# thoglu/jammy_flows

Measured on AMD Instinct MI355X. Metric: log-prob evals/sec (batch 2^20), e4+s2+e4 / gggg+f+gggg, higher is better.
Workload: dtype f32; 1 GPU; pdf("e4+s2+e4","gggg+f+gggg") log-prob, unconditional pdf with autoregressive conditioning, 1048576 rows in total, row-sharded; batch_per_gpu=1048576, total_rows=1048576, parallelism=rows sharded over 1 GPU(s)

## Files before the change

jammy_flows_amd/csrc/jf_cond_regs.h:

```cpp
#pragma once
#include <type_traits>
#include "jf_gf.h"

namespace jf {

using bf16x8 = __attribute__((ext_vector_type(8))) __bf16;
typedef __attribute__((address_space(3))) void* cs_lptr;
typedef const __attribute__((address_space(1))) void* cs_gptr;

constexpr int CS_K = 10;
constexpr int CS_HH = 4;
constexpr int CS_SLOTS = 36;
constexpr int CS_SLOT_MEAN = 0, CS_SLOT_LW = CS_K, CS_SLOT_LN = 2 * CS_K, CS_SLOT_ROT = 3 * CS_K, CS_SLOT_OFF = 3 * CS_K + CS_HH;
struct CsLayer { int hh, model_offset, inv_type; float wmin, inv_wmax, nmin, nmax; };

struct CsPackLayer { int col0, off_rot, off_mean, off_lw, off_ln, hh, model_offset; };
__device__ __forceinline__ int cs_slot_column(const CsPackLayer& o, int D, int slot, int d) {
    if (d >= D) return -1;
    if (slot < CS_SLOT_LW) return o.off_mean + slot * D + d;
    if (slot < CS_SLOT_LN) return o.off_lw + (slot - CS_SLOT_LW) * D + d;
    if (slot < CS_SLOT_ROT) return o.off_ln + (slot - CS_SLOT_LN) * D + d;
    if (slot < CS_SLOT_OFF) return (slot - CS_SLOT_ROT) < o.hh ? o.off_rot + (slot - CS_SLOT_ROT) * D + d : -1;
    if (slot == CS_SLOT_OFF) return o.model_offset ? d : -1;
    return -1;
}

__device__ __forceinline__ void cs_split(float v, __bf16& hi, __bf16& mid, __bf16& lo) {
    hi = (__bf16)v;
    const float r1 = v - (float)hi;
    mid = (__bf16)r1;
    lo = (__bf16)(r1 - (float)mid);
}

constexpr float CS_M_SCALED = 60.0f;

struct CsSums { float C, S, P, invN; };
__device__ __forceinline__ MixQ<float> cs_mixture(const float (&P)[CS_SLOTS], const CsLayer& o, float x, bool live, CsSums* sums = nullptr) {
    using Mf = M<float>;
    float iw[CS_K], wk[CS_K], u[CS_K];
    float m = INFINITY, Nn = 0.f;
#pragma unroll
    for (int k = 0; k < CS_K; ++k) {
        const float ae = o.inv_wmax + Mf::exp_fast(-P[CS_SLOT_LW + k]);
        iw[k] = ae * Mf::rcp(o.wmin * ae + 1.0f);
        wk[k] = o.nmin + o.nmax * Mf::rcp(1.0f + Mf::exp_fast(-P[CS_SLOT_LN + k]));
        u[k] = (x - P[CS_SLOT_MEAN + k]) * iw[k];
        m = fminf(m, fabsf(u[k]));
        Nn += wk[k];
    }
    const float inv = Mf::rcp(Nn);
    MixQ<float> q;
    {
        float C = 0.f, S = 0.f, Pd = 0.f;
#pragma unroll
        for (int k = 0; k < CS_K; ++k) {
            const float t = Mf::exp_fast(fminf(-u[k], 87.0f));
            const float s = Mf::rcp(1.0f + t);
            const float ts = t * s;
            C += wk[k] * s;
            S += wk[k] * ts;
            Pd += wk[k] * s * ts * iw[k];
        }
        C *= inv; S *= inv; Pd *= inv;
        q.lc = Mf::log_fast(C); q.ls = Mf::log_fast(S); q.lp = Mf::log_fast(Pd);
        q.cdf = C; q.sf = S;
        if (sums) *sums = CsSums{C, S, Pd, inv};
    }
    const bool far = m > CS_M_SCALED;
    if (!__any(live && far)) return q;
    const float em = Mf::exp_fast(-m);
    float Cu = 0.f, Cs = 0.f, Su = 0.f, Ss = 0.f, Ps = 0.f;
#pragma unroll
    for (int k = 0; k < CS_K; ++k) {
        const float t = Mf::exp_fast(m - fabsf(u[k]));
        const float hi = Mf::rcp(1.0f + t * em);
        const float c1 = wk[k] * hi, c2 = c1 * t;
        if (u[k] >= 0.f) { Cu += c1; Ss += c2; }
        else { Su += c1; Cs += c2; }
        Ps += c2 * hi * iw[k];
    }
    Cu *= inv; Cs *= inv; Su *= inv; Ss *= inv; Ps *= inv;
    if (far) {
        q.cdf = Cu + em * Cs;
        q.sf = Su + em * Ss;
        q.lc = Cu > 0.f ? Mf::log_fast(q.cdf) : Mf::log_fast(Cs) - m;
        q.ls = Su > 0.f ? Mf::log_fast(q.sf) : Mf::log_fast(Ss) - m;
        q.lp = Mf::log_fast(Ps) - m;
        if (sums) *sums = CsSums{q.cdf, q.sf, Ps * em, inv};
    }
    return q;
}

__device__ __forceinline__ void cs_derive(float (&P)[CS_SLOTS], const CsLayer& o) {
    using Mf = M<float>;
    float Nn = 0.f;
#pragma unroll
    for (int k = 0; k < CS_K; ++k) {
        const float ae = o.inv_wmax + Mf::exp_fast(-P[CS_SLOT_LW + k]);
        P[CS_SLOT_LW + k] = ae * Mf::rcp(o.wmin * ae + 1.0f);
        const float w = o.nmin + o.nmax * Mf::rcp(1.0f + Mf::exp_fast(-P[CS_SLOT_LN + k]));
        P[CS_SLOT_LN + k] = w;
        Nn += w;
    }
    const float inv = Mf::rcp(Nn);
#pragma unroll
    for (int k = 0; k < CS_K; ++k) P[CS_SLOT_LN + k] *= inv;
}

template <typename T> __device__ __forceinline__ MixQ<T> cs_mixture_derived(const T (&P)[CS_SLOTS], T x) {
    using Mf = M<T>;
    T C = T(0), S = T(0), Pd = T(0);
#pragma unroll
    for (int k = 0; k < CS_K; ++k) {
        const T iw = P[CS_SLOT_LW + k], wk = P[CS_SLOT_LN + k];
        const T u = (x - P[CS_SLOT_MEAN + k]) * iw;
        if constexpr (sizeof(T) == 4) {
            const T t = Mf::exp_fast(Mf::min(-u, T(87)));
            const T s = Mf::rcp(T(1) + t);
            const T ts = t * s;
            C += wk * s;
            S += wk * ts;
            Pd += wk * s * ts * iw;
        } else {
            const T t = Mf::exp_fast(-Mf::abs(u));
            const T hi = Mf::rcp(T(1) + t);
            const T lo = t * hi;
            const bool pos = u >= T(0);
            C += wk * (pos ? hi : lo);
            S += wk * (pos ? lo : hi);
            Pd += wk * hi * lo * iw;
        }
    }
    MixQ<T> q;
    q.lc = Mf::log_fast(C); q.ls = Mf::log_fast(S); q.lp = Mf::log_fast(Pd);
    q.cdf = C; q.sf = S;
    const bool under = !(C > Mf::TINY && S > Mf::TINY && Pd > Mf::TINY);
    if (__any(under)) {
        T m = T(INFINITY);
#pragma unroll
        for (int k = 0; k < CS_K; ++k) m = Mf::min(m, Mf::abs((x - P[CS_SLOT_MEAN + k]) * P[CS_SLOT_LW + k]));
        const T em = Mf::exp_fast(-m);
        T Cu = T(0), Cs = T(0), Su = T(0), Ss = T(0), Ps = T(0);
#pragma unroll
        for (int k = 0; k < CS_K; ++k) {
            const T iw = P[CS_SLOT_LW + k], wk = P[CS_SLOT_LN + k];
            const T u = (x - P[CS_SLOT_MEAN + k]) * iw;
            const T t = Mf::exp_fast(m - Mf::abs(u));
            const T hi = Mf::rcp(T(1) + t * em);
            const T c1 = wk * hi, c2 = c1 * t;
            if (u >= T(0)) { Cu += c1; Ss += c2; }
            else { Su += c1; Cs += c2; }
            Ps += c2 * hi * iw;
        }
        if (under) {
            q.cdf = Cu + em * Cs;
            q.sf = Su + em * Ss;
            q.lc = Cu > T(0) ? Mf::log_fast(q.cdf) : Mf::log_fast(Cs) - m;
            q.ls = Su > T(0) ? Mf::log_fast(q.sf) : Mf::log_fast(Ss) - m;
            q.lp = Mf::log_fast(Ps) - m;
        }
    }
    return q;
}

struct CsSolveInfo { int steps; bool nonconv, nonfinite; };
template <typename T, typename RSUM, typename RMAX>
__device__ __forceinline__ T cs_solve(const T (&P)[CS_SLOTS], int inv_type, bool live, T z, bool row_valid, bool leader, int32_t* status,
                                      RSUM rsum, RMAX rmax, CsSolveInfo* info = nullptr, T* logd_out = nullptr, bool have_start = false, T start = T(0)) {
    using Mf = M<T>;
    using F = typename std::conditional<sizeof(T) == 8, float, T>::type;
    T x = have_start ? start : T(0);
    if (__any(live && !have_start)) {
        F PF[CS_SLOTS];
#pragma unroll
        for (int k = 0; k < CS_SLOTS; ++k) PF[k] = k < 3 * CS_K ? (F)P[k] : F(0);
        F xf = F(0), wbar = F(0), m2 = F(0);
#pragma unroll
        for (int k = 0; k < CS_K; ++k) {
            const F pm = PF[CS_SLOT_LN + k] * PF[CS_SLOT_MEAN + k];
            xf += pm;
            m2 += pm * PF[CS_SLOT_MEAN + k];
            wbar += PF[CS_SLOT_LN + k] * M<F>::rcp(PF[CS_SLOT_LW + k]);
        }
        {
            const F zc = M<F>::min(M<F>::max((F)z, F(-8)), F(8));
            const F var_b = M<F>::max(m2 - xf * xf, F(0));
            const F sc = inv_type != JF_GF_ISIGMOID ? M<F>::sqrt(F(2.896804) * wbar * wbar + var_b) : M<F>::sqrt(wbar * wbar + F(0.30396355) * var_b);
            xf += sc * zc;
        }
#ifdef JF_PROBE_COUNT_APPROACH
        int n_ev = 0;
        xf = gf_approach<F>([&](F xx) { return cs_mixture_derived<F>(PF, xx); }, inv_type != JF_GF_ISIGMOID, (F)z, xf, live && !have_start, &n_ev);
        if (info == nullptr) { for (int i = 0; i < n_ev; ++i) status_add(status, JF_STATUS_NEWTON_STEPS, row_valid && leader); }
#else
        xf = gf_approach<F>([&](F xx) { return cs_mixture_derived<F>(PF, xx); }, inv_type != JF_GF_ISIGMOID, (F)z, xf, live && !have_start);
#endif
        if (!have_start) x = (T)xf;
    }
    bool active = row_valid;
    T ferr = T(0), prev = T(INFINITY);
    bool nonfinite = false;
    int n_steps = 0;
    T last_logd = T(0);
    bool coarse_end = false;
    for (int it = 0; it < 20 && __any(active); ++it) {
        const IcdfOut<T> s = gf_icdf<T>(inv_type, cs_mixture_derived<T>(P, x));
        const T f = s.y - z;
        T upd;
        if constexpr (sizeof(T) == 4) upd = f * Mf::exp_fast(-s.logd);
        else upd = f / Mf::exp(s.logd);
        const T usum = rsum(live ? Mf::abs(upd) : T(0));
        if (info == nullptr) status_add(status, JF_STATUS_NEWTON_STEPS, active && leader);
        n_steps += active ? 1 : 0;
        if (active) {
            const T nx = x - upd;
            if (Mf::finite(nx)) x = nx; else nonfinite = nonfinite || live;
            ferr = Mf::abs(f);
            last_logd = s.logd;
            active = usum >= newton_tol<T>();
        }
        if (sizeof(T) == 4 && !newton_reference_rule()) {
            const T xs = rsum(live ? Mf::max(Mf::abs(x), T(1)) : T(0));
            const bool done = usum < T(2.5e-7) * xs || (usum < T(JF_F32_NEWTON_FLOOR) * xs && rmax(live ? Mf::abs(f) : T(0)) <= T(1e-4));
            if (active && usum >= T(0.5) * prev && usum < T(1e-4) * xs && !done) coarse_end = true;
            if (done || (usum >= T(0.5) * prev && usum < T(1e-4) * xs)) active = false;
            prev = usum;
        }
    }
    if (logd_out != nullptr) {
        const bool stale = row_valid && (active || n_steps == 0 || coarse_end);
        if (__any(stale)) *logd_out = gf_icdf<T>(inv_type, cs_mixture_derived<T>(P, x)).logd;
        else *logd_out = last_logd;
    }
    const T prec = sizeof(T) == 8 ? T(1e-7) : T(1e-4);
    const T ferr_row = rmax(live ? ferr : T(0));
    const T nf_row = rmax(nonfinite ? T(1) : T(0));
    if (info != nullptr) {
        info->steps = n_steps; info->nonconv = ferr_row > prec; info->nonfinite = nf_row > T(0);
        return x;
    }
    status_add(status, JF_STATUS_NONCONVERGED, row_valid && leader && (ferr_row > prec));
// ... 6 lines not shown
```

jammy_flows_amd/csrc/jf_cond_split.h:

```cpp
#pragma once
#include "jf_cond_in.h"
#include "jf_cond_regs.h"
#include "jf_mfma.h"

namespace jf {

constexpr int CS_TILES = 9;
static_assert(CS_SLOTS == 4 * CS_TILES, "one register per slot, four registers per tile");
constexpr int CS_CT = 3;
constexpr int CS_CPL = CS_TILES / CS_CT;
constexpr int CS_KSTEPS = 4;
constexpr int CS_NP = 3;
constexpr int CS_FRAG = 1024;
constexpr int CS_W_BYTES = CS_CT * CS_KSTEPS * CS_NP * CS_FRAG;
constexpr int CS_B_BYTES = CS_CT * 16 * 4;
constexpr int CS_CHUNK_BYTES = CS_W_BYTES + CS_B_BYTES;
constexpr int CS_NP16 = 2;
constexpr int CS_W16_BYTES = CS_CT * CS_KSTEPS * CS_NP16 * CS_FRAG;
constexpr int CS_B16_BYTES = CS_B_BYTES + 16;
constexpr int CS_CHUNK16_BYTES = CS_W16_BYTES + CS_B16_BYTES;
constexpr float CS_H_SCALE = 16384.0f;
using f16x8 = __attribute__((ext_vector_type(8))) _Float16;
using f16x2 = __attribute__((ext_vector_type(2))) _Float16;
using f32x2 = __attribute__((ext_vector_type(2))) float;
__device__ __forceinline__ int cs_w_exponent(float wmax) {
    if (!(wmax > 0.f && wmax < INFINITY)) return 0;
    const int e = 14 - ilogbf(wmax);
    return e < -60 ? -60 : (e > 60 ? 60 : e);
}
static __global__ void __launch_bounds__(1024) cs_absmax_kernel(const float* __restrict__ W, int64_t ws, int N, int H, float* __restrict__ out) {
    __shared__ float part[16];
    float m = 0.f;
    const int lane = threadIdx.x & 63, wave = threadIdx.x >> 6;
    if (H == 128 && ws % 4 == 0 && (reinterpret_cast<uintptr_t>(W) & 15u) == 0) {
        const int half = lane >> 5, l4 = (lane & 31) * 4;
        for (int n0 = 8 * wave; n0 < N; n0 += 128) {
            f32x4 v[4];
#pragma unroll
            for (int u = 0; u < 4; ++u) {
                const int n = n0 + 2 * u + half;
                v[u] = n < N ? *reinterpret_cast<const f32x4*>(W + (int64_t)n * ws + l4) : f32x4{0.f, 0.f, 0.f, 0.f};
            }
#pragma unroll
            for (int u = 0; u < 4; ++u) m = fmaxf(fmaxf(m, fmaxf(fabsf(v[u][0]), fabsf(v[u][1]))), fmaxf(fabsf(v[u][2]), fabsf(v[u][3])));
        }
    } else {
        for (int n0 = 4 * wave; n0 < N; n0 += 64) {
            for (int k = lane; k < H; k += 64) {
                float v[4];
#pragma unroll
                for (int u = 0; u < 4; ++u) v[u] = n0 + u < N ? W[(int64_t)(n0 + u) * ws + k] : 0.f;
#pragma unroll
                for (int u = 0; u < 4; ++u) m = fmaxf(m, fabsf(v[u]));
            }
        }
    }
#pragma unroll
    for (int o = 32; o > 0; o >>= 1) m = fmaxf(m, __shfl_xor(m, o));
    if ((threadIdx.x & 63) == 0) part[threadIdx.x >> 6] = m;
    __syncthreads();
    if (threadIdx.x < 4) {
        float t = 0.f;
        if (threadIdx.x == 0) {
#pragma unroll
            for (int w = 0; w < 16; ++w) t = fmaxf(t, part[w]);
        }
        out[threadIdx.x] = t;
    }
}
template <int NP> struct CsGeom;
template <> struct CsGeom<3> { static constexpr int W = CS_W_BYTES, B = CS_B_BYTES, CHUNK = CS_CHUNK_BYTES; };
template <> struct CsGeom<2> { static constexpr int W = CS_W16_BYTES, B = CS_B16_BYTES, CHUNK = CS_CHUNK16_BYTES; };
__device__ __forceinline__ void cs_split16(float v0, float v1, unsigned& hi, unsigned& lo) {
    const f16x2 h = __builtin_convertvector(f32x2{v0, v1}, f16x2);
    const f32x2 back = __builtin_convertvector(h, f32x2);
    const f16x2 l = __builtin_convertvector(f32x2{v0 - back[0], v1 - back[1]}, f16x2);
    hi = __builtin_bit_cast(unsigned, h);
    lo = __builtin_bit_cast(unsigned, l);
}
constexpr int CS_ROWS1 = 64;
constexpr int CS_HMAX = 128, CS_K1MAX = 28;

template <typename Op> __device__ __forceinline__ float cs_rreduce(float v, Op op) {
    float a = v, b = v;
    asm("s_nop 1\n\tv_permlane16_swap_b32 %0, %1" : "+v"(a), "+v"(b));
    float c = op(a, b), e = c;
    asm("s_nop 1\n\tv_permlane32_swap_b32 %0, %1" : "+v"(c), "+v"(e));
    return op(c, e);
}
__device__ __forceinline__ float cs_rsum(float v) { return cs_rreduce(v, [](float a, float b) { return a + b; }); }
__device__ __forceinline__ float cs_rmax(float v) { return cs_rreduce(v, [](float a, float b) { return fmaxf(a, b); }); }

static inline bool cs_layer_supported(const jf_gf_layer& h, int D) {
    return h.num_kde == CS_K && h.hh_iter >= 0 && h.hh_iter <= CS_HH && h.nonlinear_stretch_type == JF_GF_STRETCH_CLASSIC &&
           h.rotation_mode == JF_GF_ROT_HOUSEHOLDER && !h.center_mean && !h.add_skewness &&
           h.width_mode == JF_GF_WIDTH_SMOOTH_SATURATION && !h.clamp_widths && h.fit_normalization && h.regulate_normalization &&
           h.width_min > 0 && h.width_max > 0 && D >= 3 && D <= 4;
}

__device__ __forceinline__ void cs_dma_chunk(__amdgpu_buffer_rsrc_t rsrc, unsigned char* dst, int g, int lane_off, int wave, int lane, int w_bytes,
                                             int b_bytes) {
#pragma unroll
    for (int u = 0; u < CS_W_BYTES / 4096; ++u)
        if (u < w_bytes / 4096) __builtin_amdgcn_raw_ptr_buffer_load_lds(rsrc, (cs_lptr)(dst + (u * 4 + wave) * 1024), 16, lane_off, g + u * 4096, 0, 0);
    if (wave == 0 && lane < b_bytes / 16) __builtin_amdgcn_raw_ptr_buffer_load_lds(rsrc, (cs_lptr)(dst + w_bytes), 16, lane * 16, g + w_bytes, 0, 0);
}

template <int RG, bool STORE_H, int NP = CS_NP>
__device__ __forceinline__ void cs_hidden(const float* __restrict__ in, int64_t in_stride, const float* __restrict__ W1, int64_t w1s,
                                          const float* __restrict__ b1, int K1, int H, int64_t row0, int64_t last, float* Xs,
                                          bf16x8 (&hB)[RG][CS_KSTEPS][NP], float* __restrict__ h_out, int64_t hs, const CondIn* cin = nullptr) {
    using MF = Mfma16<float>;
    constexpr int CS_ROWS = CS_ROWS1 * RG;
    constexpr int MT = 16, KS = 4, NREG = 4, JH = CS_HMAX / MT;
    const int tid = threadIdx.x, lane = tid & 63, wave = tid >> 6;
    const int li = lane & 15, lq = lane >> 4;
    const int k1p = (K1 + KS - 1) / KS * KS, ldk = k1p + 1;
    float* W1s = Xs + CS_ROWS * ldk;
    float* b1s = W1s + CS_HMAX * ldk;
    {
        const int nx = CS_ROWS * k1p, nw = CS_HMAX * k1p;
        if (cin) {
            const bool any_embed = cond_in_any_embed(*cin);
            for (int base = 0; base < nx; base += 4 * 256) {
                CondLoc<float> loc[4]; float va[4], vb[4]; int o[4]; bool keep[4];
#pragma unroll
                for (int u = 0; u < 4; ++u) {
                    const int idx = base + u * 256 + tid;
                    const int r = idx / k1p, c = idx - r * k1p;
                    const int64_t gr = row0 + r;
                    loc[u] = cond_in_locate<float>(*cin, gr <= last ? gr : last, c < K1 ? c : 0);
                    keep[u] = c < K1;
                    o[u] = idx < nx ? r * ldk + c : -1;
                }
#pragma unroll
                for (int u = 0; u < 4; ++u) { va[u] = *loc[u].pa; vb[u] = *loc[u].pb; }
#pragma unroll
                for (int u = 0; u < 4; ++u) {
                    const float t = cond_in_finish<float, true>(loc[u], va[u], vb[u], any_embed);
                    if (o[u] >= 0) Xs[o[u]] = keep[u] ? t : 0.f;
                }
            }
        } else
        for (int base = 0; base < nx; base += 4 * 256) {
            float v[4]; int o[4];
#pragma unroll
            for (int u = 0; u < 4; ++u) {
                const int idx = base + u * 256 + tid;
                const int r = idx / k1p, c = idx - r * k1p;
                const int64_t gr = row0 + r;
                const float t = in[(gr <= last ? gr : last) * in_stride + (c < K1 ? c : 0)];
                v[u] = c < K1 ? t : 0.f;
                o[u] = idx < nx ? r * ldk + c : -1;
            }
#pragma unroll
            for (int u = 0; u < 4; ++u) if (o[u] >= 0) Xs[o[u]] = v[u];
        }
        for (int base = 0; base < nw; base += 4 * 256) {
            float v[4]; int o[4];
#pragma unroll
            for (int u = 0; u < 4; ++u) {
                const int idx = base + u * 256 + tid;
                const int r = idx / k1p, c = idx - r * k1p;
                const float t = W1[(int64_t)(r < H ? r : H - 1) * w1s + (c < K1 ? c : 0)];
                v[u] = (r < H && c < K1) ? t : 0.f;
                o[u] = idx < nw ? r * ldk + c : -1;
            }
#pragma unroll
            for (int u = 0; u < 4; ++u) if (o[u] >= 0) W1s[o[u]] = v[u];
        }
        if (tid < CS_HMAX) b1s[tid] = tid < H ? b1[tid < H ? tid : 0] : 0.f;
    }
    __syncthreads();
#pragma unroll
    for (int g = 0; g < RG; ++g) {
        typename MF::Acc acc[JH];
#pragma unroll
        for (int j = 0; j < JH; ++j)
#pragma unroll
            for (int r = 0; r < NREG; ++r) acc[j][r] = 0.f;
        for (int s = 0; s < k1p / KS; ++s) {
            const int kk = s * KS + lq;
            const float xb = Xs[((wave * RG + g) * MT + li) * ldk + kk];
#pragma unroll
            for (int j = 0; j < JH; ++j) acc[j] = MF::mma(W1s[(j * MT + li) * ldk + kk], xb, acc[j]);
        }
#pragma unroll
        for (int s = 0; s < CS_KSTEPS; ++s) {
            using u32x4 = __attribute__((ext_vector_type(4))) unsigned;
            u32x4 q0, q1, q2;
#pragma unroll
            for (int i = 0; i < 8; i += 2) {
                const int j = 2 * s + (i >> 2), r = i & 3;
                const float h0 = M<float>::tanh_fast(acc[j][r] + b1s[j * MT + 4 * lq + r]);
                const float h1 = M<float>::tanh_fast(acc[j][r + 1] + b1s[j * MT + 4 * lq + r + 1]);
                if constexpr (STORE_H) { acc[j][r] = h0; acc[j][r + 1] = h1; }
                if constexpr (NP == 2) {
                    unsigned ph, pl;
                    cs_split16(h0 * CS_H_SCALE, h1 * CS_H_SCALE, ph, pl);
                    q0[i >> 1] = ph; q1[i >> 1] = pl;
                    continue;
                }
                const unsigned a0 = __builtin_bit_cast(unsigned, h0), a1 = __builtin_bit_cast(unsigned, h1);
                const float r0 = h0 - __builtin_bit_cast(float, a0 & 0xffff0000u), r1 = h1 - __builtin_bit_cast(float, a1 & 0xffff0000u);
                const unsigned c0 = __builtin_bit_cast(unsigned, r0), c1 = __builtin_bit_cast(unsigned, r1);
                const float s0 = r0 - __builtin_bit_cast(float, c0 & 0xffff0000u), s1 = r1 - __builtin_bit_cast(float, c1 & 0xffff0000u);
                q0[i >> 1] = __builtin_amdgcn_perm(a1, a0, 0x07060302u);
                q1[i >> 1] = __builtin_amdgcn_perm(c1, c0, 0x07060302u);
                q2[i >> 1] = __builtin_amdgcn_perm(__builtin_bit_cast(unsigned, s1), __builtin_bit_cast(unsigned, s0), 0x07060302u);
            }
            hB[g][s][0] = __builtin_bit_cast(bf16x8, q0); hB[g][s][1] = __builtin_bit_cast(bf16x8, q1);
            if constexpr (NP == 3) hB[g][s][2] = __builtin_bit_cast(bf16x8, q2);
        }
        if constexpr (STORE_H) {
            const int64_t r = row0 + (wave * RG + g) * MT + li;
            if (r <= last) {
#pragma unroll
                for (int j = 0; j < JH; ++j) {
                    const int c = j * MT + 4 * lq;
                    if (c < H) *reinterpret_cast<f32x4*>(h_out + r * hs + c) = acc[j];
                }
            }
        }
    }
}

}
```

jammy_flows_amd/csrc/jf_cond_split_kernel.h:

```cpp
#pragma once
#include "jf_cond_split.h"

namespace jf {

constexpr int CS_MAX_PRE = 4;
struct CsArgs {
    const float* in; int64_t in_stride;
    const float* W1; int64_t w1s; const float* b1;
    const unsigned char* packed;
    int K1, H;
    const float* x; int64_t xs;
    const float* ld_in;
    int64_t B;
    int D, n_layers;
    CsLayer L[JF_MAX_CHAIN];
    float* x_out; int64_t xos;
    float* ld_out;
    const float* blp_in; float* blp_out;
    int32_t* status;
    float* aux;
    CondIn cin;
    const float* ld_pre[CS_MAX_PRE]; const float* blp_pre[CS_MAX_PRE];
    int n_ld_pre, n_blp_pre;
    float* total;
};

template <int RG, bool FWD, bool SAVE, int NP>
__device__ __forceinline__ void cond_gf_split_body(const CsArgs& a, const int block, unsigned char* smem_raw) {
    using G = CsGeom<NP>;
    constexpr int CS_ROWS = CS_ROWS1 * RG;
    constexpr int MT = 16;
    unsigned char* Ws0 = smem_raw;
    float* Xs = reinterpret_cast<float*>(smem_raw + G::CHUNK);
    const int tid = threadIdx.x, lane = tid & 63, wave = tid >> 6;
    const int li = lane & 15, lq = lane >> 4;
    const int64_t row0 = (int64_t)block * CS_ROWS;
    const int64_t last = a.B - 1;
    const int D = a.D;
    const __amdgpu_buffer_rsrc_t packed_rsrc =
        __builtin_amdgcn_make_buffer_rsrc(const_cast<unsigned char*>(a.packed), 0, a.n_layers * CS_CPL * G::CHUNK, 0x00027000);
    const int lane_off = wave * 1024 + lane * 16;
    auto dma = [&](int chunk) {
        const int img = FWD ? (a.n_layers - 1 - chunk / CS_CPL) * CS_CPL + chunk % CS_CPL : chunk;
        const int g = img * G::CHUNK;
        cs_dma_chunk(packed_rsrc, Ws0 + (chunk & 1) * G::CHUNK, g, lane_off, wave, lane, G::W, G::B);
    };
    dma(0);

    bf16x8 hB[RG][CS_KSTEPS][NP];
    cs_hidden<RG, false, NP>(a.in, a.in_stride, a.W1, a.w1s, a.b1, a.K1, a.H, row0, last, Xs, hB, nullptr, 0, a.cin.n ? &a.cin : nullptr);
    const bool live = lq < D, leader = lq == 0;
    int d = live ? lq : D - 1;
    int64_t row[RG]; bool row_valid[RG];
    float x[RG], ld[RG];
#pragma unroll
    for (int g = 0; g < RG; ++g) {
        row[g] = row0 + (wave * RG + g) * MT + li;
        row_valid[g] = row[g] <= last;
        const int64_t rrow = row_valid[g] ? row[g] : last;
        x[g] = a.x[rrow * a.xs + d];
        ld[g] = a.ld_in ? a.ld_in[rrow] : 0.f;
    }

    auto landed = [&]() { asm volatile("s_waitcnt vmcnt(0) lgkmcnt(0)\n\ts_barrier" ::: "memory"); };

    const int n_chunks = a.n_layers * CS_CPL;
    landed();
    int chunk = 0;
    for (int li = 0; li < a.n_layers; ++li) {
        const int l = FWD ? li : a.n_layers - 1 - li;
        float P[RG][CS_SLOTS];
#pragma unroll
        for (int c = 0; c < CS_CPL; ++c, ++chunk) {
            if (chunk + 1 < n_chunks) dma(chunk + 1);
            const unsigned char* Ws = Ws0 + (chunk & 1) * G::CHUNK;
            const float* Bs = reinterpret_cast<const float*>(Ws + G::W);
            f32x4 acc[RG][CS_CT];
#pragma unroll
            for (int t = 0; t < CS_CT; ++t) {
                const f32x4 bias = *reinterpret_cast<const f32x4*>(Bs + t * 16 + 4 * lq);
#pragma unroll
                for (int g = 0; g < RG; ++g) acc[g][t] = bias;
            }
            bf16x8 A[2][CS_CT][NP];
            auto load_a = [&](int s, int buf) {
#pragma unroll
                for (int t = 0; t < CS_CT; ++t)
#pragma unroll
                    for (int p = 0; p < NP; ++p)
                        A[buf][t][p] = *reinterpret_cast<const bf16x8*>(Ws + ((t * CS_KSTEPS + s) * NP + p) * CS_FRAG + lane * 16);
            };
            load_a(0, 0);
#pragma unroll
            for (int s = 0; s < CS_KSTEPS; ++s) {
                const int b = s & 1;
                if (s + 1 < CS_KSTEPS) load_a(s + 1, b ^ 1);
                if constexpr (NP == 3) {
                    constexpr int PA[6] = {2, 1, 0, 1, 0, 0}, PB[6] = {0, 1, 2, 0, 1, 0};
#pragma unroll
                    for (int i = 0; i < 6; ++i)
#pragma unroll
                        for (int t = 0; t < CS_CT; ++t)
#pragma unroll
                            for (int g = 0; g < RG; ++g)
                                acc[g][t] = __builtin_amdgcn_mfma_f32_16x16x32_bf16(A[b][t][PA[i]], hB[g][s][PB[i]], acc[g][t], 0, 0, 0);
                } else {
#pragma unroll
                    for (int i = 0; i < 3; ++i)
#pragma unroll
                        for (int t = 0; t < CS_CT; ++t)
#pragma unroll
                            for (int g = 0; g < RG; ++g) {
                                const f16x8 af = __builtin_bit_cast(f16x8, A[b][t][i == 0 ? 1 : 0]), bf = __builtin_bit_cast(f16x8, hB[g][s][i == 1 ? 1 : 0]);
                                acc[g][t] = __builtin_amdgcn_mfma_f32_16x16x32_f16(af, bf, acc[g][t], 0, 0, 0);
                            }
                }
            }
            if constexpr (NP == 3) {
#pragma unroll
                for (int g = 0; g < RG; ++g)
#pragma unroll
                    for (int t = 0; t < CS_CT; ++t)
#pragma unroll
                        for (int r = 0; r < 4; ++r) P[g][4 * (c * CS_CT + t) + r] = acc[g][t][r];
            } else {
                const float inv = Bs[CS_B_BYTES / 4];
#pragma unroll
                for (int g = 0; g < RG; ++g)
#pragma unroll
                    for (int t = 0; t < CS_CT; ++t)
#pragma unroll
                        for (int r = 0; r < 4; ++r) P[g][4 * (c * CS_CT + t) + r] = acc[g][t][r] * inv;
            }
            if (c + 1 < CS_CPL) landed();
        }
        const CsLayer o = a.L[l];
#pragma unroll
        for (int g = 0; g < RG; ++g) {
            if constexpr (!FWD) {
                float xg = x[g] - P[g][CS_SLOT_OFF];
#pragma unroll
                for (int i = 0; i < CS_HH; ++i) {
                    if (i < o.hh) {
                        const float v = live ? P[g][CS_SLOT_ROT + i] : 0.f;
                        const float n2 = cs_rsum(v * v), dot = cs_rsum(v * xg);
                        xg -= 2.0f * dot * M<float>::rcp(n2) * v;
                    }
                }
                CsSums sums;
                const MixQ<float> q = cs_mixture(P[g], o, xg, live, SAVE ? &sums : nullptr);
                if constexpr (SAVE) {
                    {
                        int t2 = tid;
                        asm volatile("" : "+v"(t2));
                        row[g] = row0 + ((t2 >> 6) * RG + g) * MT + (t2 & 15);
                        row_valid[g] = row[g] <= last;
                    }
                    if (row_valid[g]) {
                        const int64_t slot = ((int64_t)l * a.B + row[g]) * 4 + lq;
                        reinterpret_cast<f32x4*>(a.aux)[slot] = f32x4{sums.C, sums.S, sums.P, sums.invN};
                        a.aux[(int64_t)a.n_layers * a.B * 16 + slot] = x[g];
                    }
                }
                const IcdfOut<float> sy = gf_icdf<float>(o.inv_type, q);
                x[g] = sy.y;
                ld[g] += cs_rsum(live ? sy.logd : 0.f);
            } else {
                cs_derive(P[g], o);
                float slogd;
                float xs = cs_solve<float>(P[g], o.inv_type, live, x[g], row_valid[g], leader, a.status, [](float v) { return cs_rsum(v); },
                                    [](float v) { return cs_rmax(v); }, nullptr, &slogd);
                ld[g] -= cs_rsum(live ? slogd : 0.f);
#pragma unroll
                for (int i = CS_HH - 1; i >= 0; --i) {
                    if (i < o.hh) {
                        const float v = live ? P[g][CS_SLOT_ROT + i] : 0.f;
                        const float n2 = cs_rsum(v * v), dot = cs_rsum(v * xs);
                        xs -= 2.0f * dot * M<float>::rcp(n2) * v;
                    }
                }
                x[g] = xs + P[g][CS_SLOT_OFF];
            }
        }
        landed();
    }

    if constexpr (!FWD) {
        int t2 = tid;
        asm volatile("" : "+v"(t2));
        const int lane2 = t2 & 63, wave2 = t2 >> 6, li2 = lane2 & 15, lq2 = lane2 >> 4;
        d = lq2 < D ? lq2 : D - 1;
#pragma unroll
        for (int g = 0; g < RG; ++g) {
            row[g] = row0 + (wave2 * RG + g) * MT + li2;
            row_valid[g] = row[g] <= last;
        }
    }
#pragma unroll
    for (int g = 0; g < RG; ++g) {
        if (row_valid[g] && live) a.x_out[row[g] * a.xos + d] = x[g];
        if constexpr (FWD) {
            if (row_valid[g] && leader) a.ld_out[row[g]] = ld[g];
        } else {
            float sb = 0.f;
            if (a.blp_out) sb = cs_rsum(live ? -0.5f * x[g] * x[g] - M<float>::HALF_LN_2PI : 0.f);
            if (row_valid[g] && leader) {
                float ldv = ld[g], bv = sb + (a.blp_in ? a.blp_in[row[g]] : 0.f);
                if (a.n_ld_pre > 0) {
                    float t = a.ld_pre[0][row[g]];
                    for (int i = 1; i < a.n_ld_pre; ++i) t += a.ld_pre[i][row[g]];
                    ldv = t + ldv;
                }
                if (a.n_blp_pre > 0) {
                    float t = a.blp_pre[0][row[g]];
                    for (int i = 1; i < a.n_blp_pre; ++i) t += a.blp_pre[i][row[g]];
                    bv = t + bv;
                }
                a.ld_out[row[g]] = ldv;
                if (a.blp_out) a.blp_out[row[g]] = bv;
                if (a.total) a.total[row[g]] = bv + ldv;
            }
            const float bad = cs_rmax((live && !M<float>::finite(x[g])) ? 1.f : 0.f);
            status_add(a.status, JF_STATUS_NONFINITE, row_valid[g] && leader && (bad > 0.f || !M<float>::finite(ld[g])));
        }
    }
}

}
```

jammy_flows_amd/csrc/jf_gf.h:

```cpp
#pragma once
#include "jf_common.h"
#include "jf_math.h"
#include "jf_spline.h"

namespace jf {

template <typename T> struct GfLayerDev {
    int K, hh, model_offset, fit_norm, reg_norm, inv_type, width_mode, clamp_widths;
    int fast;
    int stretch;
    int off_box;
    int n_params;
    int col0;
    int off_rot, off_mean, off_lw, off_ln;
    int vec_ok;
    int rot_mode, center_mean, skew;
    int off_skew;
    T wmin, wmax, inv_wmax, nmin, nmax, lw_lo, lw_hi;
};

constexpr double PADE_BOUND = 0.5e-7;
constexpr double PADE_A = 0.147;

template <typename T> __device__ __forceinline__ T gf_inv_width(const GfLayerDev<T>& o, T x) {
    if (o.width_mode == JF_GF_WIDTH_SMOOTH_SATURATION) {
        if (o.clamp_widths) x = clampv(x, o.lw_lo, o.lw_hi);
        const T ae = o.inv_wmax + M<T>::exp_fast(-x);
        return ae * M<T>::rcp(o.wmin * ae + T(1));
    }
    if (o.clamp_widths) x = clampv(x, o.lw_lo, o.lw_hi);
    if (o.width_mode == JF_GF_WIDTH_EXP) return M<T>::rcp(M<T>::exp(x) + o.wmin);
    return M<T>::rcp(softplus(x) + o.wmin);
}
template <typename T> __device__ __forceinline__ T gf_width(const GfLayerDev<T>& o, T x) {
    if (o.width_mode == JF_GF_WIDTH_SMOOTH_SATURATION) {
        if (o.clamp_widths) x = clampv(x, o.lw_lo, o.lw_hi);
        return o.wmin + M<T>::rcp(o.inv_wmax + M<T>::exp_fast(-x));
    }
    if (o.clamp_widths) x = clampv(x, o.lw_lo, o.lw_hi);
    if (o.width_mode == JF_GF_WIDTH_EXP) return M<T>::exp(x) + o.wmin;
    return softplus(x) + o.wmin;
}

template <typename T> __device__ __forceinline__ void gf_derive_column(T* __restrict__ row, const GfLayerDev<T>& o, int D, int d) {
    const int K = o.K;
    T nsum = T(0), nmax = T(0);
    if (o.fit_norm && !o.reg_norm) {
        nmax = row[o.off_ln + d];
        for (int k = 1; k < K; ++k) nmax = M<T>::max(nmax, row[o.off_ln + k * D + d]);
    }
    for (int k = 0; k < K; ++k) {
        const int i = k * D + d;
        row[o.off_lw + i] = M<T>::rcp(gf_width(o, row[o.off_lw + i]));
        if (o.fit_norm) {
            const T xn = row[o.off_ln + i];
            const T w = o.reg_norm ? o.nmin + o.nmax * M<T>::rcp(T(1) + M<T>::exp_fast(-xn)) : M<T>::exp(xn - nmax);
            row[o.off_ln + i] = w;
            nsum += w;
        }
    }
    if (o.fit_norm) {
        const T inv = M<T>::rcp(nsum);
        for (int k = 0; k < K; ++k) row[o.off_ln + k * D + d] *= inv;
    }
}

template <typename T> __device__ __forceinline__ T gf_weight(const GfLayerDev<T>& o, T xn, T shift) {
    return o.reg_norm ? o.nmin + o.nmax * M<T>::rcp(T(1) + M<T>::exp_fast(-xn)) : M<T>::exp(xn - shift);
}

template <typename T> __device__ __forceinline__ void gf_derive_reflection(T* __restrict__ row, const GfLayerDev<T>& o, int D, int i) {
    T n2 = T(0);
    for (int d = 0; d < D; ++d) { const T v = row[o.off_rot + i * D + d]; n2 += v * v; }
    const T s = M<T>::SQRT2 / M<T>::sqrt(n2);
    for (int d = 0; d < D; ++d) row[o.off_rot + i * D + d] *= s;
}

template <typename T> struct MixQ { T lc, ls, lp, cdf, sf; };

template <typename T> struct Pade { T F2, F2mF; };

template <typename T> __device__ __forceinline__ Pade<T> pade_terms(const MixQ<T>& q) {
    const T a = T(PADE_A);
    const T c = T(2.0 / (3.14159265358979323846 * PADE_A));
    const T dlt = q.sf - q.cdf;
    Pade<T> p;
    if constexpr (sizeof(T) == 4) {
        const bool centre = M<T>::min(q.cdf, q.sf) > T(0.01);
        T ln_fac = q.lc + q.ls + T(1.38629436111989061883);
        if (__any(centre)) {
            const T l1p = M<T>::log1p(-dlt * dlt);
            ln_fac = centre ? l1p : ln_fac;
        }
        const T F = ln_fac * T(0.5) + c;
        const T rad = -ln_fac * T(1.0 / PADE_A);
        p.F2 = M<T>::sqrt_fast(F * F + rad);
        p.F2mF = F > T(0) ? rad * M<T>::rcp(p.F2 + F) : p.F2 - F;
        return p;
    }
    const T ln_fac = (M<T>::min(q.cdf, q.sf) > T(0.01)) ? M<T>::log1p(-dlt * dlt) : q.lc + q.ls + T(1.38629436111989061883);
    const T F = ln_fac * T(0.5) + c;
    const T rad = -ln_fac / a;
    p.F2 = M<T>::sqrt(F * F + rad);
    p.F2mF = F > T(0) ? rad / (p.F2 + F) : p.F2 - F;
    return p;
}
template <typename T> __device__ __forceinline__ T pade_value(const Pade<T>& p) {
    if constexpr (sizeof(T) == 4) return M<T>::sqrt_fast(M<T>::max(T(2) * p.F2mF, T(0)));
    return M<T>::sqrt(M<T>::max(T(2) * p.F2mF, T(0)));
}
template <typename T> __device__ __forceinline__ T pade_logderiv(const Pade<T>& p, const MixQ<T>& q) {
    if constexpr (sizeof(T) == 4) {
        const T log_num = M<T>::log_fast(p.F2mF + T(1.0 / PADE_A));
        const T log_den = T(1.03972077083991796413) + T(0.5) * M<T>::log_fast(p.F2mF) + M<T>::log_fast(p.F2);
        return log_num - log_den - q.ls - q.lc + M<T>::log_fast(M<T>::abs(q.sf - q.cdf));
    }
    const T log_num = M<T>::log(p.F2mF + T(1.0 / PADE_A));
    const T log_den = T(1.03972077083991796413) + T(0.5) * M<T>::log(p.F2mF) + M<T>::log(p.F2);
    return log_num - log_den - q.ls - q.lc + M<T>::log(M<T>::abs(q.sf - q.cdf));
}

__device__ __forceinline__ float inormal_central_f32(const MixQ<float>& q) {
    const float w = fmaxf(-(q.lc + q.ls + 1.38629436112f), 0.0f);
    const bool c = w < 5.0f;
    const float t = c ? w - 2.5f : M<float>::sqrt_fast(w) - 3.0f;
    float p = c ? 2.81022636e-08f : -0.000200214257f;
    p = fmaf(p, t, c ? 3.43273939e-07f : 0.000100950558f);
    p = fmaf(p, t, c ? -3.5233877e-06f : 0.00134934322f);
    p = fmaf(p, t, c ? -4.39150654e-06f : -0.00367342844f);
    p = fmaf(p, t, c ? 0.00021858087f : 0.00573950773f);
    p = fmaf(p, t, c ? -0.00125372503f : -0.0076224613f);
    p = fmaf(p, t, c ? -0.00417768164f : 0.00943887047f);
    p = fmaf(p, t, c ? 0.246640727f : 1.00167406f);
    p = fmaf(p, t, c ? 1.50140941f : 2.83297682f);
    return 1.41421356237f * p * (q.cdf - q.sf);
}
template <typename T> __device__ __forceinline__ T inormal_central_f32(const MixQ<T>&) { return T(0); }

template <typename T> __device__ __forceinline__ T gf_inverse_cdf(int inv_type, const MixQ<T>& q, T& logd) {
    if (inv_type == JF_GF_ISIGMOID) {
        logd = q.lp - q.lc - q.ls;
        return q.lc - q.ls;
    }
    const T bound = T(PADE_BOUND);
    if (inv_type == JF_GF_INORMAL_FULL_PADE) {
        const Pade<T> p = pade_terms(q);
        const T tot = pade_value(p);
        const bool centre = (q.cdf > T(0.49999)) && (q.cdf < T(0.50001));
        logd = centre ? T(0.91893852361801185) + q.lp : pade_logderiv(p, q) + q.lp;
        return q.cdf <= q.sf ? -tot : tot;
    }
    const bool left = q.cdf <= bound, right = q.sf <= bound;
    if (!left && !right) {
        if constexpr (sizeof(T) == 4) {
            const T y = inormal_central_f32(q);
            logd = M<T>::HALF_LN_2PI + T(0.5) * y * y + q.lp;
            return y;
        } else {
            const T e = M<T>::erfcinv(T(2) * M<T>::min(q.cdf, q.sf));
            logd = M<T>::HALF_LN_2PI + e * e + q.lp;
            return (q.cdf < q.sf ? -M<T>::SQRT2 : M<T>::SQRT2) * e;
        }
    }
    T tot;
    if (inv_type == JF_GF_INORMAL_PARTLY_CRUDE) {
        const T lsum = q.lc + q.ls;
        if constexpr (sizeof(T) == 4) {
            tot = M<T>::sqrt_fast(T(-2) * lsum) - T(0.4717);
            logd = T(-0.5) * M<T>::log_fast(T(-2) * lsum) - lsum + q.lp;
        } else {
            tot = M<T>::sqrt(T(-2) * lsum) - T(0.4717);
            logd = T(-0.5) * M<T>::log(T(-2) * lsum) - lsum + q.lp;
        }
    } else {
        const Pade<T> p = pade_terms(q);
        tot = pade_value(p);
        logd = pade_logderiv(p, q) + q.lp;
    }
    return right ? tot : -tot;
}

template <typename T> struct IcdfOut { T y, logd; };
template <typename T> __device__ __forceinline__ IcdfOut<T> gf_icdf(int inv_type, MixQ<T> q) {
    IcdfOut<T> r;
    r.y = gf_inverse_cdf<T>(inv_type, q, r.logd);
    return r;
}
template <> __device__ __noinline__ IcdfOut<double> gf_icdf<double>(int inv_type, MixQ<double> q) {
    IcdfOut<double> r;
    r.y = gf_inverse_cdf<double>(inv_type, q, r.logd);
    return r;
}

template <int CTRL> __device__ __forceinline__ float dpp_swap(float v) {
    return __builtin_bit_cast(float, __builtin_amdgcn_update_dpp(0, __builtin_bit_cast(int, v), CTRL, 0xf, 0xf, true));
}
template <int CTRL> __device__ __forceinline__ double dpp_swap(double v) {
    const long long b = __builtin_bit_cast(long long, v);
    const int lo = __builtin_amdgcn_update_dpp(0, (int)(b & 0xffffffffll), CTRL, 0xf, 0xf, true);
    const int hi = __builtin_amdgcn_update_dpp(0, (int)(b >> 32), CTRL, 0xf, 0xf, true);
    return __builtin_bit_cast(double, ((long long)hi << 32) | (long long)(unsigned)lo);
}
constexpr int DPP_XOR1 = 0xB1;
constexpr int DPP_XOR2 = 0x4E;
constexpr int DPP_HALF_MIRROR = 0x141;

constexpr int DPP_ROW_ROR8 = 0x128;

template <typename T> __device__ __forceinline__ T xor16(T v) { return __shfl_xor(v, 16, 64); }
template <typename T> __device__ __forceinline__ T xor32(T v) { return __shfl_xor(v, 32, 64); }

template <typename T, int G> __device__ __forceinline__ T group_sum(T v) {
    if constexpr (G >= 2) v += dpp_swap<DPP_XOR1>(v);
    if constexpr (G >= 4) v += dpp_swap<DPP_XOR2>(v);
    if constexpr (G >= 8) v += dpp_swap<DPP_HALF_MIRROR>(v);
    if constexpr (G >= 16) v += dpp_swap<DPP_ROW_ROR8>(v);
    if constexpr (G >= 32) v += xor16(v);
    if constexpr (G >= 64) v += xor32(v);
    return v;
}
template <typename T, int G> __device__ __forceinline__ T group_max(T v) {
    if constexpr (G >= 2) v = M<T>::max(v, dpp_swap<DPP_XOR1>(v));
    if constexpr (G >= 4) v = M<T>::max(v, dpp_swap<DPP_XOR2>(v));
    if constexpr (G >= 8) v = M<T>::max(v, dpp_swap<DPP_HALF_MIRROR>(v));
    if constexpr (G >= 16) v = M<T>::max(v, dpp_swap<DPP_ROW_ROR8>(v));
    if constexpr (G >= 32) v = M<T>::max(v, xor16(v));
    if constexpr (G >= 64) v = M<T>::max(v, xor32(v));
    return v;
}

template <typename T, int G, bool RAW> __device__ __forceinline__ T gfg_reflect(const T* __restrict__ p, int off, bool live, T x) {
    const T v = live ? p[off] : T(0);
    if constexpr (RAW) {
        const T n2 = group_sum<T, G>(v * v), dot = group_sum<T, G>(v * x);
        return x - T(2) * dot * M<T>::rcp(n2) * v;
    } else {
        return x - v * group_sum<T, G>(v * x);
    }
}
template <typename T, int G, bool RAW> __device__ __forceinline__ T gfg_rotate_inv(const T* __restrict__ p, const GfLayerDev<T>& o, int D, bool live, T x) {
    for (int i = 0; i < o.hh; ++i) x = gfg_reflect<T, G, RAW>(p, o.off_rot + i * D, live, x);
    return x;
}
template <typename T, int G, bool RAW> __device__ __forceinline__ T gfg_rotate_fwd(const T* __restrict__ p, const GfLayerDev<T>& o, int D, bool live, T x) {
    for (int i = o.hh - 1; i >= 0; --i) x = gfg_reflect<T, G, RAW>(p, o.off_rot + i * D, live, x);
    return x;
}


template <typename T, bool RAW> __device__ __forceinline__ MixQ<T> gfg_mixture_scaled(const T* __restrict__ p, const GfLayerDev<T>& o, int D, T x, T shift) {
    const T uniform_w = RAW ? T(1) : M<T>::rcp(T(o.K));
    T m = T(INFINITY);
    for (int k = 0; k < o.K; ++k) {
        const T iw = RAW ? gf_inv_width(o, p[o.off_lw + k * D]) : p[o.off_lw + k * D];
        m = M<T>::min(m, M<T>::abs((x - p[o.off_mean + k * D]) * iw));
    }
    const T em = M<T>::exp_fast(-m);
    T Cu = T(0), Cs = T(0), Su = T(0), Ss = T(0), Ps = T(0), Nn = T(0);
    for (int k = 0; k < o.K; ++k) {
        const T iw = RAW ? gf_inv_width(o, p[o.off_lw + k * D]) : p[o.off_lw + k * D];
        const T wk = o.fit_norm ? (RAW ? gf_weight(o, p[o.off_ln + k * D], shift) : p[o.off_ln + k * D]) : uniform_w;
        const T u = (x - p[o.off_mean + k * D]) * iw;
        const T t = M<T>::exp_fast(m - M<T>::abs(u));
        const T hi = M<T>::rcp(T(1) + t * em);
        const T c1 = wk * hi, c2 = c1 * t;
        if (u >= T(0)) { Cu += c1; Ss += c2; }
        else { Su += c1; Cs += c2; }
        Ps += c2 * hi * iw;
        Nn += wk;
    }
    if constexpr (RAW) {
        const T inv = M<T>::rcp(Nn);
        Cu *= inv; Cs *= inv; Su *= inv; Ss *= inv; Ps *= inv;
    }
    MixQ<T> q;
    q.cdf = Cu + em * Cs;
    q.sf = Su + em * Ss;
    q.lc = Cu > T(0) ? M<T>::log_fast(q.cdf) : M<T>::log_fast(Cs) - m;
    q.ls = Su > T(0) ? M<T>::log_fast(q.sf) : M<T>::log_fast(Ss) - m;
    q.lp = M<T>::log_fast(Ps) - m;
    return q;
}

template <typename T, bool RAW, bool FAST> __device__ __forceinline__ MixQ<T> gfg_mixture_impl(const T* __restrict__ p, const GfLayerDev<T>& o, int D, T x) {
    T C = T(0), S = T(0), P = T(0), Nn = T(0), shift = T(0);
    const bool fit_norm = FAST ? true : (o.fit_norm != 0);
    const T uniform_w = RAW ? T(1) : M<T>::rcp(T(o.K));
    if (!FAST && RAW && o.fit_norm && !o.reg_norm) {
        shift = p[o.off_ln];
        for (int k = 1; k < o.K; ++k) shift = M<T>::max(shift, p[o.off_ln + k * D]);
    }
    const T* pm = p + o.off_mean;
    const T* pw = p + o.off_lw;
    const T* pn = p + o.off_ln;
#pragma unroll 2
    for (int k = 0; k < o.K; ++k) {
        const T mu = pm[k * D], rw = pw[k * D];
        const T rn = fit_norm ? pn[k * D] : T(0);
        T iw, wk;
        if constexpr (RAW) {
            if constexpr (FAST) {
                const T ae = o.inv_wmax + M<T>::exp_fast(-rw);
                iw = ae * M<T>::rcp(o.wmin * ae + T(1));
                wk = o.nmin + o.nmax * M<T>::rcp(T(1) + M<T>::exp_fast(-rn));
            } else {
                iw = gf_inv_width(o, rw);
                wk = fit_norm ? gf_weight(o, rn, shift) : T(1);
            }
        } else {
            iw = rw;
            wk = fit_norm ? rn : uniform_w;
        }
        const T u = (x - mu) * iw;
        const T t = M<T>::exp_fast(-M<T>::abs(u));
        const T hi = M<T>::rcp(T(1) + t);
        const T lo = t * hi;
        const bool pos = u >= T(0);
        C += wk * (pos ? hi : lo);
        S += wk * (pos ? lo : hi);
        P += wk * hi * lo * iw;
        if constexpr (RAW) Nn += wk;
    }
    if constexpr (RAW) {
        const T inv = M<T>::rcp(Nn);
        C *= inv; S *= inv; P *= inv;
    }
    MixQ<T> q;
    q.lc = M<T>::log_fast(C); q.ls = M<T>::log_fast(S); q.lp = M<T>::log_fast(P);
// ... 125 lines not shown
```

Before: 1.652 billion log-prob evals/s.

## Fold projection scale into mixture math and batch Householder norm reductions

In the inverse path, the per-chunk multiply of MFMA accumulators by the projection scale is dropped. The scale is instead folded into the mixture evaluation, which now uses native base-2 exp/log with the constants pre-multiplied. The four Householder vector norms are computed with a single batched cross-lane reduction (cs_rsum4) instead of one reduction per reflection. The Pade inverse CDF skips the log1p centre branch and uses the ln(4·C·S) form, which is algebraically equivalent when C+S=1. The aim is fewer VALU ops, fewer permlane reductions and less divergence, at the cost of slightly different rounding and losing the dead-lane zeroing of the rotation vectors.

After: 1.695 billion log-prob evals/s, median of 6. 2.6% higher.

```diff
diff --git a/jammy_flows_amd/csrc/jf_cond_regs.h b/jammy_flows_amd/csrc/jf_cond_regs.h
--- a/jammy_flows_amd/csrc/jf_cond_regs.h
+++ b/jammy_flows_amd/csrc/jf_cond_regs.h
@@ -35,58 +35,66 @@
 constexpr float CS_M_SCALED = 60.0f;
 
 struct CsSums { float C, S, P, invN; };
-__device__ __forceinline__ MixQ<float> cs_mixture(const float (&P)[CS_SLOTS], const CsLayer& o, float x, bool live, CsSums* sums = nullptr) {
+constexpr float CS_LOG2E = 1.44269504088896340736f, CS_LN2 = 0.69314718055994530942f, CS_LNLN2 = -0.36651292058166432701f;
+__device__ __forceinline__ float cs_exp2(float x) { return __builtin_amdgcn_exp2f(x); }
+__device__ __forceinline__ float cs_log2(float x) { return __builtin_amdgcn_logf(x); }
+__device__ __forceinline__ float cs_uniform(float x) { return __builtin_bit_cast(float, __builtin_amdgcn_readfirstlane(__builtin_bit_cast(int, x))); }
+__device__ __forceinline__ MixQ<float> cs_mixture(const float (&A)[CS_SLOTS], const CsLayer& o, float pscale, float x, bool live,
+                                                  CsSums* sums = nullptr) {
     using Mf = M<float>;
+    const float ke = cs_uniform(-pscale * CS_LOG2E);
+    const float iwmax2 = cs_uniform(o.inv_wmax * CS_LOG2E), wmin2 = cs_uniform(o.wmin * CS_LN2);
     float iw[CS_K], wk[CS_K], u[CS_K];
-    float m = INFINITY, Nn = 0.f;
-#pragma unroll
-    for (int k = 0; k < CS_K; ++k) {
-        const float ae = o.inv_wmax + Mf::exp_fast(-P[CS_SLOT_LW + k]);
-        iw[k] = ae * Mf::rcp(o.wmin * ae + 1.0f);
-        wk[k] = o.nmin + o.nmax * Mf::rcp(1.0f + Mf::exp_fast(-P[CS_SLOT_LN + k]));
-        u[k] = (x - P[CS_SLOT_MEAN + k]) * iw[k];
-        m = fminf(m, fabsf(u[k]));
-        Nn += wk[k];
+    float m, Nn;
+#pragma unroll
+    for (int k = 0; k < CS_K; ++k) {
+        const float ae = fmaf(cs_exp2(A[CS_SLOT_LW + k] * ke), CS_LOG2E, iwmax2);
+        iw[k] = ae * Mf::rcp(fmaf(wmin2, ae, 1.0f));
+        wk[k] = o.nmin + o.nmax * Mf::rcp(1.0f + cs_exp2(A[CS_SLOT_LN + k] * ke));
+        u[k] = fmaf(-A[CS_SLOT_MEAN + k], pscale, x) * iw[k];
+        m = k ? fminf(m, fabsf(u[k])) : fabsf(u[k]);
+        Nn = k ? Nn + wk[k] : wk[k];
     }
     const float inv = Mf::rcp(Nn);
     MixQ<float> q;
     {
-        float C = 0.f, S = 0.f, Pd = 0.f;
+        float C, S, Pd;
 #pragma unroll
         for (int k = 0; k < CS_K; ++k) {
-            const float t = Mf::exp_fast(fminf(-u[k], 87.0f));
+            const float t = cs_exp2(fminf(-u[k], 87.0f * CS_LOG2E));
             const float s = Mf::rcp(1.0f + t);
             const float ts = t * s;
-            C += wk[k] * s;
-            S += wk[k] * ts;
-            Pd += wk[k] * s * ts * iw[k];
+            const float ws = wk[k] * s;
+            C = k ? C + ws : ws;
+            S = k ? fmaf(wk[k], ts, S) : wk[k] * ts;
+            Pd = k ? fmaf(ws * ts, iw[k], Pd) : ws * ts * iw[k];
         }
         C *= inv; S *= inv; Pd *= inv;
-        q.lc = Mf::log_fast(C); q.ls = Mf::log_fast(S); q.lp = Mf::log_fast(Pd);
+        q.lc = Mf::log_fast(C); q.ls = Mf::log_fast(S); q.lp = fmaf(cs_log2(Pd), CS_LN2, CS_LNLN2);
         q.cdf = C; q.sf = S;
-        if (sums) *sums = CsSums{C, S, Pd, inv};
-    }
-    const bool far = m > CS_M_SCALED;
+        if (sums) *sums = CsSums{C, S, Pd * CS_LN2, inv};
+    }
+    const bool far = m > CS_M_SCALED * CS_LOG2E;
     if (!__any(live && far)) return q;
-    const float em = Mf::exp_fast(-m);
-    float Cu = 0.f, Cs = 0.f, Su = 0.f, Ss = 0.f, Ps = 0.f;
-#pragma unroll
-    for (int k = 0; k < CS_K; ++k) {
-        const float t = Mf::exp_fast(m - fabsf(u[k]));
+    const float em = cs_exp2(-m);
+    float Cu = 0.f, Cs = 0.f, Su = 0.f, Ss = 0.f, Ps;
+#pragma unroll
+    for (int k = 0; k < CS_K; ++k) {
+        const float t = cs_exp2(m - fabsf(u[k]));
         const float hi = Mf::rcp(1.0f + t * em);
         const float c1 = wk[k] * hi, c2 = c1 * t;
         if (u[k] >= 0.f) { Cu += c1; Ss += c2; }
         else { Su += c1; Cs += c2; }
-        Ps += c2 * hi * iw[k];
+        Ps = k ? fmaf(c2 * hi, iw[k], Ps) : c2 * hi * iw[k];
     }
     Cu *= inv; Cs *= inv; Su *= inv; Ss *= inv; Ps *= inv;
     if (far) {
         q.cdf = Cu + em * Cs;
         q.sf = Su + em * Ss;
-        q.lc = Cu > 0.f ? Mf::log_fast(q.cdf) : Mf::log_fast(Cs) - m;
-        q.ls = Su > 0.f ? Mf::log_fast(q.sf) : Mf::log_fast(Ss) - m;
-        q.lp = Mf::log_fast(Ps) - m;
-        if (sums) *sums = CsSums{q.cdf, q.sf, Ps * em, inv};
+        q.lc = Cu > 0.f ? Mf::log_fast(q.cdf) : CS_LN2 * (cs_log2(Cs) - m);
+        q.ls = Su > 0.f ? Mf::log_fast(q.sf) : CS_LN2 * (cs_log2(Ss) - m);
+        q.lp = fmaf(cs_log2(Ps) - m, CS_LN2, CS_LNLN2);
+        if (sums) *sums = CsSums{q.cdf, q.sf, Ps * CS_LN2 * em, inv};
     }
     return q;
 }
diff --git a/jammy_flows_amd/csrc/jf_cond_split.h b/jammy_flows_amd/csrc/jf_cond_split.h
--- a/jammy_flows_amd/csrc/jf_cond_split.h
+++ b/jammy_flows_amd/csrc/jf_cond_split.h
@@ -89,6 +89,16 @@
     return op(c, e);
 }
 __device__ __forceinline__ float cs_rsum(float v) { return cs_rreduce(v, [](float a, float b) { return a + b; }); }
+template <typename F> __device__ __forceinline__ void cs_rsum4(float a, float b, float c, float d, F f, float (&out)[4]) {
+    asm("s_nop 1\n\tv_permlane16_swap_b32 %0, %1\n\tv_permlane16_swap_b32 %2, %3" : "+v"(a), "+v"(b), "+v"(c), "+v"(d));
+    float ab = a + b, cd = c + d;
+    asm("s_nop 1\n\tv_permlane32_swap_b32 %0, %1" : "+v"(ab), "+v"(cd));
+    float t = f(ab + cd), t2 = t;
+    asm("s_nop 1\n\tv_permlane32_swap_b32 %0, %1" : "+v"(t), "+v"(t2));
+    float t1 = t, t3 = t2;
+    asm("s_nop 1\n\tv_permlane16_swap_b32 %0, %1\n\tv_permlane16_swap_b32 %2, %3" : "+v"(t), "+v"(t1), "+v"(t2), "+v"(t3));
+    out[0] = t; out[1] = t1; out[2] = t2; out[3] = t3;
+}
 __device__ __forceinline__ float cs_rmax(float v) { return cs_rreduce(v, [](float a, float b) { return fmaxf(a, b); }); }
 
 static inline bool cs_layer_supported(const jf_gf_layer& h, int D) {
diff --git a/jammy_flows_amd/csrc/jf_cond_split_kernel.h b/jammy_flows_amd/csrc/jf_cond_split_kernel.h
--- a/jammy_flows_amd/csrc/jf_cond_split_kernel.h
+++ b/jammy_flows_amd/csrc/jf_cond_split_kernel.h
@@ -70,6 +70,7 @@
     for (int li = 0; li < a.n_layers; ++li) {
         const int l = FWD ? li : a.n_layers - 1 - li;
         float P[RG][CS_SLOTS];
+        float pscale = 1.0f;
 #pragma unroll
         for (int c = 0; c < CS_CPL; ++c, ++chunk) {
             if (chunk + 1 < n_chunks) dma(chunk + 1);
@@ -125,12 +126,13 @@
                         for (int r = 0; r < 4; ++r) P[g][4 * (c * CS_CT + t) + r] = acc[g][t][r];
             } else {
                 const float inv = Bs[CS_B_BYTES / 4];
+                if constexpr (!FWD) pscale = cs_uniform(inv);
 #pragma unroll
                 for (int g = 0; g < RG; ++g)
 #pragma unroll
                     for (int t = 0; t < CS_CT; ++t)
 #pragma unroll
-                        for (int r = 0; r < 4; ++r) P[g][4 * (c * CS_CT + t) + r] = acc[g][t][r] * inv;
+                        for (int r = 0; r < 4; ++r) P[g][4 * (c * CS_CT + t) + r] = FWD ? acc[g][t][r] * inv : acc[g][t][r];
             }
             if (c + 1 < CS_CPL) landed();
         }
@@ -138,17 +140,16 @@
 #pragma unroll
         for (int g = 0; g < RG; ++g) {
             if constexpr (!FWD) {
-                float xg = x[g] - P[g][CS_SLOT_OFF];
+                float xg = fmaf(-P[g][CS_SLOT_OFF], pscale, x[g]);
+                const float* v = &P[g][CS_SLOT_ROT];
+                float r2[CS_HH];
+                cs_rsum4(v[0] * v[0], v[1] * v[1], v[2] * v[2], v[3] * v[3], [](float n2) { return 2.0f * M<float>::rcp(n2); }, r2);
 #pragma unroll
                 for (int i = 0; i < CS_HH; ++i) {
-                    if (i < o.hh) {
-                        const float v = live ? P[g][CS_SLOT_ROT + i] : 0.f;
-                        const float n2 = cs_rsum(v * v), dot = cs_rsum(v * xg);
-                        xg -= 2.0f * dot * M<float>::rcp(n2) * v;
-                    }
+                    if (i < o.hh) xg -= cs_rsum(v[i] * xg) * r2[i] * v[i];
                 }
                 CsSums sums;
-                const MixQ<float> q = cs_mixture(P[g], o, xg, live, SAVE ? &sums : nullptr);
+                const MixQ<float> q = cs_mixture(P[g], o, pscale, xg, live, SAVE ? &sums : nullptr);
                 if constexpr (SAVE) {
                     {
                         int t2 = tid;
diff --git a/jammy_flows_amd/csrc/jf_gf.h b/jammy_flows_amd/csrc/jf_gf.h
--- a/jammy_flows_amd/csrc/jf_gf.h
+++ b/jammy_flows_amd/csrc/jf_gf.h
@@ -80,7 +80,7 @@
 
 template <typename T> struct Pade { T F2, F2mF; };
 
-template <typename T> __device__ __forceinline__ Pade<T> pade_terms(const MixQ<T>& q) {
+template <typename T, bool TAIL = false> __device__ __forceinline__ Pade<T> pade_terms(const MixQ<T>& q) {
     const T a = T(PADE_A);
     const T c = T(2.0 / (3.14159265358979323846 * PADE_A));
     const T dlt = q.sf - q.cdf;
@@ -88,7 +88,7 @@
     if constexpr (sizeof(T) == 4) {
         const bool centre = M<T>::min(q.cdf, q.sf) > T(0.01);
         T ln_fac = q.lc + q.ls + T(1.38629436111989061883);
-        if (__any(centre)) {
+        if (!TAIL && __any(centre)) {
             const T l1p = M<T>::log1p(-dlt * dlt);
             ln_fac = centre ? l1p : ln_fac;
         }
@@ -98,7 +98,7 @@
         p.F2mF = F > T(0) ? rad * M<T>::rcp(p.F2 + F) : p.F2 - F;
         return p;
     }
-    const T ln_fac = (M<T>::min(q.cdf, q.sf) > T(0.01)) ? M<T>::log1p(-dlt * dlt) : q.lc + q.ls + T(1.38629436111989061883);
+    const T ln_fac = (!TAIL && M<T>::min(q.cdf, q.sf) > T(0.01)) ? M<T>::log1p(-dlt * dlt) : q.lc + q.ls + T(1.38629436111989061883);
     const T F = ln_fac * T(0.5) + c;
     const T rad = -ln_fac / a;
     p.F2 = M<T>::sqrt(F * F + rad);
@@ -173,7 +173,7 @@
             logd = T(-0.5) * M<T>::log(T(-2) * lsum) - lsum + q.lp;
         }
     } else {
-        const Pade<T> p = pade_terms(q);
+        const Pade<T> p = pade_terms<T, true>(q);
         tot = pade_value(p);
         logd = pade_logderiv(p, q) + q.lp;
     }
```
